# Plachtaa/FAcodec

Hardware: NVIDIA B200
Metric: audio_seconds_per_second (higher is better)
Workload: dtype f32 I/O and accumulation; every product is a 3-MMA split of fp32 operands: fp16 hi + 2^11-scaled fp16 lo (22 mantissa bits, register-promoted accumulation) upstream of the VQ, bf16 hi + bf16 lo (16 bits) downstream

## Files before the change

facodec_b200/csrc/engine.cu:

```cuda
#include <cmath>
#include <cstdio>
#include <cstdlib>
#include <cstring>
#include <map>
#include <string>
#include <vector>

#include "../../include/facodec_b200.h"
#include "../../include/facodec_b200_debug.h"
#include "common.cuh"
#include "kernels.h"

using namespace fac;

namespace {

constexpr int HOP = 300;
constexpr int LATENT = 1024;
constexpr int N_FFT = 2048;
constexpr int WIN = 1200;
constexpr int N_BINS = 1025;
constexpr int SPEC_LD = 2052;
constexpr int SPEC_TC_LD = 2176;
constexpr int N_MELS = 80;

struct HostTensor {
    std::vector<float> data;
    std::vector<int64_t> shape;
    size_t numel() const { size_t n = 1; for (auto s : shape) n *= (size_t)s; return n; }
};

struct ConvW {
    size_t w = 0, b = 0; int Cin = 0, Cout = 0, K = 1, ldw = 0;
    bool tc = false; size_t tcw = 0; int vf = 1, Kr = 0, tcN = 0;
    bool promoted = false;
    bool has16 = false; size_t tcw16 = 0;
    bool has_f16s = false; size_t tcw_f16s = 0;
    bool has_tt = false; size_t tcw_tt = 0;
};
struct SnakeW { size_t a = 0, ia = 0; int C = 0; };
struct LstmW { ConvW ih[2]; size_t whh[2] = {0, 0}; size_t whh16[2] = {0, 0}; bool has16 = false; int H = 0, U = 0, G = 0;
               size_t whh2[2][2] = {{0, 0}, {0, 0}}; bool has2[2] = {false, false}; };
struct ResW { SnakeW s1; ConvW c7; SnakeW s2; ConvW c1; int dil = 1; };
struct VqW { size_t w_in, b_in, cb, cbn, cbn2, w_out, b_out; };

struct EncW {
    ConvW conv0;
    struct Block { ResW res[3]; SnakeW snake; ConvW down; int stride; } blk[4];
    LstmW lstm; SnakeW snake; ConvW conv_out;
};
struct DecW {
    ConvW conv0; LstmW lstm;
    struct Block { SnakeW snake; ConvW up; int stride; int cout; ResW res[3]; } blk[4];
    SnakeW snake; ConvW conv_out;
    bool causal = true, has_lstm = true;
};
struct RedW {
    size_t emb_p = 0, emb_c[2] = {0, 0};
    ConvW cond, wn_in[16], wn_rs[16], conv_out;
    int hidden = 512, layers = 16;
};
struct QuantW {
    VqW vq[6];
    ConvW spec0, spec3, glu[2], cq, ck, cv, co, fc, timbre_linear;
    ConvW mel_lin, wn_in[8], wn_rs[8], mel_lin2;
    ConvW dft; size_t fb = 0;
    ConvW dft_tc;
};
struct RvqSet { int nq; VqW vq[8]; };

}

struct fac_handle {
    int device = 0;
    std::string err;
    std::map<std::string, HostTensor> host[FAC_NUM_MODULES];
    bool have[FAC_NUM_MODULES] = {false, false, false, false, false};
    bool finalized = false;
    std::vector<float> pack;
    float* warena = nullptr; size_t wfloats = 0;
    EncW enc; DecW dec; QuantW qw;
    RedW red; DecW dec2;
    std::vector<RvqSet> rvqs; std::vector<float*> rvq_arenas;
    struct Stream;
    std::vector<Stream*> streams;
    struct HeadSet;
    std::vector<HeadSet*> heads;
    char* ws = nullptr; size_t ws_bytes = 0;
    int launches = 0;
    int use_tc = 2;
    int fuse_res = 1;
    int lstm_v2 = 1;
    int dec_lstm_fp16 = 1;
    int enc_mufu = 0;
    int attn_stream = 0;
    int dec_c7_f16 = 1;
    int enc_tt = 1;
    int enc_f16 = 0;
    int tc_occ2 = 256;
    bool dec_bf16 = true;
    int overlap_front = 1; cudaStream_t side = nullptr; cudaEvent_t ev_fork = nullptr, ev_join = nullptr;
    float* aa_filter = nullptr;
    float* mel16_arena = nullptr; ConvW mel16_dft, mel16_dft_tc; size_t mel16_fb = 0;
    struct LossScale { ConvW dft; size_t fb = 0; int s = 0, nfft = 0, nb = 0, ld = 0; };
    float* loss_arena = nullptr; LossScale loss_scale[6];
    struct SpecScale { ConvW dft; size_t fb = 0; int w = 0, nb = 0, ld = 0, n_out = 0; bool mel = false; };
    float* spec_arena = nullptr; std::vector<SpecScale> spec_scales; std::vector<double> spec_key;
    bool profiling = false;
    struct ProfRec { std::string name; cudaEvent_t a, b; double flops, bytes; };
    std::vector<ProfRec> prof;
    struct ProfAgg { double ms = 0, flops = 0, bytes = 0; long launches = 0; };
    std::map<std::string, ProfAgg> prof_agg;
    std::map<std::string, std::pair<float*, size_t>> taps;
};

struct fac_handle::Stream {
    int B = 0;
    bool alive = false;
    long long enc_samples = 0, dec_frames = 0;
    float* x_hist = nullptr; int x_hist_len = 0;
    float* ey_hist = nullptr; int ey_hist_len = 0;
    float* z_hist = nullptr; int z_hist_len = 0;
    float* dy_hist = nullptr; int dy_hist_len = 0;
    uint32_t* enc_h[2] = {nullptr, nullptr}; float* enc_c[2] = {nullptr, nullptr};
    uint32_t* dec_h[2] = {nullptr, nullptr}; float* dec_c[2] = {nullptr, nullptr};
    void* all[12] = {nullptr};
};

struct fac_handle::HeadSet {
    int indim = 0, outdim = 0, nheads = 0, global_pred = 0;
    struct Unit { size_t a1, b1, a2, b2; ConvW c7, c1; int dil; } unit[3];
    size_t af, bf;
    ConvW lin[8];
    std::map<std::string, HostTensor> staged;
    float* arena = nullptr;
    bool ready = false;
};

namespace {

size_t pack_alloc(fac_handle* h, size_t n) {
    size_t off = (h->pack.size() + 63) / 64 * 64;
    h->pack.resize(off + n, 0.f);
    return off;
}

const HostTensor* find(fac_handle* h, int m, const std::string& k) {
    auto it = h->host[m].find(k);
    return it == h->host[m].end() ? nullptr : &it->second;
}

struct PackError { std::string msg; };
const HostTensor& need(fac_handle* h, int m, const std::string& k) {
    const HostTensor* t = find(h, m, k);
    if (!t) throw PackError{"missing tensor '" + k + "' in module " + std::to_string(m)};
    return *t;
}

std::vector<float> folded_weight(fac_handle* h, int m, const std::string& prefix, std::vector<int64_t>& shape) {
    if (const HostTensor* w = find(h, m, prefix + ".weight")) {
        shape = w->shape;
        return w->data;
    }
    const HostTensor& v = need(h, m, prefix + ".weight_v");
    const HostTensor& g = need(h, m, prefix + ".weight_g");
    shape = v.shape;
    size_t d0 = (size_t)v.shape[0], inner = v.numel() / d0;
    if (g.numel() != d0) throw PackError{"weight_g shape mismatch at " + prefix};
    std::vector<float> w(v.numel());
    for (size_t i = 0; i < d0; ++i) {
        double s = 0.0;
        for (size_t j = 0; j < inner; ++j) { double x = v.data[i * inner + j]; s += x * x; }
        float scale = g.data[i] / (float)std::sqrt(s);
        for (size_t j = 0; j < inner; ++j) w[i * inner + j] = v.data[i * inner + j] * scale;
    }
// ... 491 lines not shown
    p.res = o.res; p.valid_len = o.valid_len;
    p.B = B; p.Tin = Tin; p.Cin = w.Cin; p.Tout = Tout; p.Cout = w.Cout;
    p.K = w.K; p.dil = o.dil; p.stride = o.stride;
    p.pad_left = o.pad_left; p.pad_right = o.pad_right; p.pad_reflect = o.reflect;
    p.ldw = w.ldw; p.ldy = o.ldy ? o.ldy : w.Cout; p.ldx = o.ldx ? o.ldx : w.Cin;
    p.y_transposed = o.transposed;
    p.x_bstride = (size_t)Tin * p.ldx;
    p.y_bstride = (size_t)Tout * p.ldy;
    double flops = 2.0 * B * Tout * (double)w.Cout * w.K * w.Cin;
    double bytes = 4.0 * ((double)B * Tin * w.Cin + (double)B * Tout * w.Cout * (o.res ? 2 : 1) + (double)w.K * w.Cin * w.Cout);
    char det[96];
    snprintf(det, sizeof det, "%s Cin%d Cout%d K%d d%d T%d", name, w.Cin, w.Cout, w.K, o.dil, Tout);
    c.begin("conv", flops, bytes, det);
    c.check(launch_conv(p, c.st), name);
    c.end();
}

int sconv(Ctx& c, const ConvW& w, const float* x, float* y, int B, int T, int dil, int stride, ConvOpts o,
          const char* name, bool causal = true) {
    int k_eff = (w.K - 1) * dil + 1;
    o.dil = dil; o.stride = stride;
    const int total = k_eff - stride, extra = conv_extra_pad(T, k_eff, stride);
    o.pad_left = causal ? total : total - total / 2;
    o.pad_right = (causal ? 0 : total / 2) + extra;
    o.reflect = 1;
    int Tout = conv_out_len(T, k_eff, stride);
    run_conv(c, w, x, y, B, T, Tout, o, name);
    return Tout;
}

bool residual_unit_fused(Ctx& c, const ResW& r, const float* x, float* y, int B, int T, bool causal) {
    if (c.h->use_tc < 1 || !c.h->fuse_res || c.vq_critical || !r.c7.tc || !r.c1.tc || r.c7.promoted || r.c1.promoted ||
        r.c7.Cin != r.c7.Cout || r.c1.K != 1 || r.c7.vf != 1)
        return false;
    TcConvParams tp;
    tp.Cin = r.c7.Cin; tp.Cout = r.c7.Cout; tp.vf = 1; tp.Kr = r.c7.K; tp.dil = r.dil; tp.fused = 1;
    tp.bf16 = (c.h->dec_bf16 && r.c7.has16 && r.c1.has16) ? 1 : 0;
    tp.g1f16 = (tp.bf16 && r.c7.has_f16s && c.h->dec_c7_f16) ? 1 : 0;
    tp.occ2_maxn = c.h->tc_occ2;
    tp.Tout = T;
    if (c.h->fuse_res == 2 && r.c7.Cout > 128) return false;
    if (!tc_conv_plan(tp)) return false;
    if (c.dry) return true;
    const int k_eff = (r.c7.K - 1) * r.dil + 1;
    tp.x = x; tp.y = y; tp.res = x;
    tp.wblob = c.W(tp.g1f16 ? r.c7.tcw_f16s : (tp.bf16 ? r.c7.tcw16 : r.c7.tcw)); tp.bias = c.W(r.c7.b);
    tp.wblob2 = c.W(tp.bf16 ? r.c1.tcw16 : r.c1.tcw); tp.bias2 = c.W(r.c1.b);
    tp.in_alpha = c.W(r.s1.a); tp.in_inv_alpha = c.W(r.s1.ia);
    tp.out_act = ACT_SNAKE; tp.out_alpha = c.W(r.s2.a); tp.out_inv_alpha = c.W(r.s2.ia);
    tp.B = B; tp.Tin = T; tp.ldx = r.c7.Cin;
    const int pl = causal ? k_eff - 1 : (k_eff - 1) - (k_eff - 1) / 2;
    tp.PLr = pl; tp.pad_left_s = pl; tp.pad_right_s = k_eff - 1 - pl; tp.reflect = 1;
    tp.Tout = T; tp.ldy = r.c7.Cout;
    tp.x_bstride = (size_t)T * r.c7.Cin; tp.y_bstride = (size_t)T * r.c7.Cout;
    double flops = 2.0 * B * T * (double)r.c7.Cout * r.c7.Cin * (r.c7.K + 1);
    double bytes = 4.0 * ((double)B * T * r.c7.Cin * 2 + (double)B * T * r.c7.Cout + (double)(r.c7.K + 1) * r.c7.Cin * r.c7.Cout);
    char det[96];
    snprintf(det, sizeof det, "res.fused C%d K%d d%d T%d", r.c7.Cin, r.c7.K, r.dil, T);
    c.begin("conv_tc", flops, bytes, det);
    c.check(launch_conv_tc(tp, c.st), "res.fused");
    c.end();
    return true;
}

void residual_unit(Ctx& c, const ResW& r, const float* x, float* tmp, float* y, int B, int T, bool causal = true) {
    if (residual_unit_fused(c, r, x, y, B, T, causal)) return;
    ConvOpts o1;
    o1.in_snake = &r.s1;
    o1.out_snake = &r.s2;
    sconv(c, r.c7, x, tmp, B, T, r.dil, 1, o1, "res.conv7", causal);
    ConvOpts o2;
    o2.res = x;
    sconv(c, r.c1, tmp, y, B, T, 1, 1, o2, "res.conv1", causal);
}

struct LstmState { uint32_t* h[2] = {nullptr, nullptr}; float* c[2] = {nullptr, nullptr}; };

void slstm(Ctx& c, const LstmW& L, const float* x, float* y, int B, int T, LstmState* st = nullptr) {
    const int H = L.H;
    float* xg = c.alloc<float>((size_t)B * T * 4 * H);
    float* h1 = c.alloc<float>((size_t)B * T * H);
    float* hT = c.alloc<float>((size_t)2 * H * 32);
    uint32_t* h16 = c.alloc<uint32_t>((size_t)2 * 2 * (H / 2) * 32);
    unsigned int* bar = c.alloc<unsigned int>(64);
    for (int l = 0; l < 2; ++l) {
        const float* in = l == 0 ? x : h1;
        ConvOpts o;
        run_conv(c, L.ih[l], in, xg, 1, B * T, B * T, o, "lstm.ih");
        if (c.dry) continue;
        const int pass3 = (c.vq_critical || !c.h->dec_bf16) ? 1 : 0;
        const bool v2 = c.h->lstm_v2 && L.has2[pass3] && (pass3 || c.h->dec_lstm_fp16);
        for (int b0 = 0; b0 < B; b0 += 32) {
            int nb = B - b0 < 32 ? B - b0 : 32;
            LstmParams p;
            p.xg = xg + (size_t)b0 * T * 4 * H;
            p.whh_p = c.W(L.whh[l]);
            if (c.h->dec_bf16 && L.has16 && !c.vq_critical) { p.bf16 = 1; p.whh_p16 = c.W(L.whh16[l]); }
            p.skip = l == 1 ? x + (size_t)b0 * T * H : nullptr;
            p.y = (l == 0 ? h1 : y) + (size_t)b0 * T * H;
            p.hT = hT; p.bar = bar;
            p.B = nb; p.T = T; p.H = H; p.U = L.U; p.G = L.G;
            c.begin("lstm_rec", 2.0 * nb * T * 4.0 * H * H, 4.0 * ((double)nb * T * 5 * H + 4.0 * H * H));
            if (st && (!v2 || B > 32)) { c.check(cudaErrorNotSupported, "lstm.stream (needs the resident-W kernel and B <= 32)"); c.end(); continue; }
            if (v2) {
                p.whh_p2 = reinterpret_cast<const uint32_t*>(c.W(L.whh2[l][pass3]));
                p.h16 = h16; p.pass3 = pass3;
                if (st) { p.state_h = st->h[l]; p.state_c = st->c[l]; }
                c.check(launch_lstm2_layer(p, c.st), "lstm.rec2");
            } else {
                c.check(launch_lstm_layer(p, c.st), "lstm.rec");
            }
            c.end();
        }
    }
}

size_t enc_stage_floats(int B, int T) {
    return (size_t)B * ((size_t)T + 16) * 64;
}

float* encoder_front(Ctx& c, const float* x, int B, int T, int* frames) {
    const EncW& e = c.h->enc;
    size_t stage = enc_stage_floats(B, T);
    float* buf[3] = {c.alloc<float>(stage), c.alloc<float>(stage), c.alloc<float>(stage)};
    int cur = 0;
    int t = sconv(c, e.conv0, x, buf[0], B, T, 1, 1, ConvOpts(), "enc.conv0");
    c.tap("enc_conv0", buf[0], (size_t)B * t * 64);
    static const char* blk_names[4] = {"enc_block1", "enc_block2", "enc_block3", "enc_block4"};
    for (int i = 0; i < 4; ++i) {
        for (int j = 0; j < 3; ++j) {
            int tmp = (cur + 1) % 3, nxt = (cur + 2) % 3;
            residual_unit(c, e.blk[i].res[j], buf[cur], buf[tmp], buf[nxt], B, t);
            cur = nxt;
        }
        ConvOpts o;
        o.in_snake = &e.blk[i].snake;
        int nxt = (cur + 1) % 3;
        t = sconv(c, e.blk[i].down, buf[cur], buf[nxt], B, t, 1, e.blk[i].stride, o, "enc.down");
        cur = nxt;
        c.tap(blk_names[i], buf[cur], (size_t)B * t * e.blk[i].down.Cout);
    }
    *frames = t;
    return buf[cur];
}

int encoder_forward(Ctx& c, const float* x, int B, int T, float* z_out, bool z_nct) {
    const EncW& e = c.h->enc;
    c.vq_critical = true;
    int t = 0;
    float* feats = encoder_front(c, x, B, T, &t);
    float* ylstm = c.alloc<float>((size_t)B * t * LATENT);
    slstm(c, e.lstm, feats, ylstm, B, t);
    c.tap("enc_lstm", ylstm, (size_t)B * t * 1024);
    ConvOpts o;
    o.in_snake = &e.snake;
    if (z_nct) {
        float* zcl = c.alloc<float>((size_t)B * t * LATENT);
        sconv(c, e.conv_out, ylstm, zcl, B, t, 1, 1, o, "enc.conv_out");
        if (!c.dry) c.check(launch_transpose(zcl, z_out, B, t, LATENT, c.st), "enc.z_T");
    } else {
        sconv(c, e.conv_out, ylstm, z_out, B, t, 1, 1, o, "enc.conv_out");
    }
    c.vq_critical = false;
    return t;
}

size_t decoder_stage_floats(int B, int Tf) {
    size_t stage = (size_t)B * (size_t)Tf * 28800 + 1024;
    size_t first = (size_t)B * Tf * 1536;
    return first > stage ? first : stage;
}
void decoder_stack(Ctx& c, const DecW& d, const float* in, int in_idx, float* const* buf, int B, int Tf, float* y) {
    int t = Tf;
    const float* cur_p = in;
    int cur = in_idx;
    static const char* dblk_names[4] = {"dec_block1", "dec_block2", "dec_block3", "dec_block4"};
    for (int i = 0; i < 4; ++i) {
        ConvOpts o;
        o.in_snake = &d.blk[i].snake;
        o.pad_left = 1; o.pad_right = d.causal ? 0 : 1; o.reflect = 0;
        int nxt = cur < 0 ? 0 : (cur + 1) % 3;
        run_conv(c, d.blk[i].up, cur_p, buf[nxt], B, t, t, o, "dec.up");
        cur = nxt; cur_p = buf[cur];
        t *= d.blk[i].stride;
        for (int j = 0; j < 3; ++j) {
            int tmp = (cur + 1) % 3, nx2 = (cur + 2) % 3;
            residual_unit(c, d.blk[i].res[j], buf[cur], buf[tmp], buf[nx2], B, t, d.causal);
            cur = nx2; cur_p = buf[cur];
        }
// ... 1150 lines not shown
        auto i0 = [](double v) { double s = 1, t = 1; for (int k = 1; k < 60; ++k) { t *= (v / (2 * k)) * (v / (2 * k)); s += t; } return s; };
        float f[12];
        double sum = 0;
        double tmp[12];
        for (int i = 0; i < ks; ++i) {
            double r = 2.0 * i / (ks - 1) - 1.0;
            double w = i0(beta_k * std::sqrt(std::max(0.0, 1 - r * r))) / i0(beta_k);
            double tm = (i - half) + 0.5;
            double xx = 2 * cutoff * tm;
            double sinc = xx == 0 ? 1.0 : std::sin(M_PI * xx) / (M_PI * xx);
            tmp[i] = 2 * cutoff * w * sinc;
            sum += tmp[i];
        }
        for (int i = 0; i < ks; ++i) f[i] = (float)(tmp[i] / sum);
        cudaError_t e = cudaMalloc(&h->aa_filter, sizeof(f));
        if (e == cudaSuccess) e = cudaMemcpy(h->aa_filter, f, sizeof(f), cudaMemcpyHostToDevice);
        if (e != cudaSuccess) { h->err = cudaGetErrorString(e); cudaGetLastError(); return FAC_ERR_CUDA; }
    }
    return FAC_OK;
}

int fac_alias_free_act(fac_handle* h, const float* x, int B, int C, int T, int act, const float* alpha,
                       const float* beta, float* y, void* stream) {
    if (!h || !x || !y || B <= 0 || C <= 0 || T <= 0 || (act == 1 && (!alpha || !beta))) return FAC_ERR_INVALID;
    int rc0 = ensure_aa_filter(h);
    if (rc0) return rc0;
    cudaError_t e = launch_alias_free_act(x, y, B, C, T, h->aa_filter, act == 1 ? alpha : nullptr, act == 1 ? beta : nullptr,
                                          (cudaStream_t)stream);
    if (e != cudaSuccess) { h->err = cudaGetErrorString(e); return FAC_ERR_CUDA; }
    return FAC_OK;
}

int fac_debug_conv(fac_handle* h, const float* x, const float* w_host, const float* bias_host, int B, int Tin, int Cin,
                   int Cout, int K, int dil, int stride, int pad_left, int pad_right, int reflect,
                   const float* in_alpha_host, const float* out_alpha_host, int act, const float* res, float* y,
                   int Tout, void* stream) {
    if (!h || !x || !w_host || !y) return FAC_ERR_INVALID;
    cudaSetDevice(h->device);
    cudaStream_t st = (cudaStream_t)stream;
    int ldw = (Cout + 3) / 4 * 4;
    std::vector<float> pk((size_t)K * Cin * ldw + Cout + 2 * Cin + 2 * Cout + 96, 0.f);
    for (int co = 0; co < Cout; ++co)
        for (int ci = 0; ci < Cin; ++ci)
            for (int k = 0; k < K; ++k) pk[((size_t)k * Cin + ci) * ldw + co] = w_host[((size_t)co * Cin + ci) * K + k];
    auto al4 = [](size_t v) { return (v + 3) / 4 * 4; };
    size_t o_b = (size_t)K * Cin * ldw, o_ia = al4(o_b + Cout), o_iia = al4(o_ia + Cin), o_oa = al4(o_iia + Cin), o_oia = al4(o_oa + Cout);
    for (int i = 0; i < Cout; ++i) pk[o_b + i] = bias_host ? bias_host[i] : 0.f;
    for (int i = 0; i < Cin; ++i) { pk[o_ia + i] = in_alpha_host ? in_alpha_host[i] : 1.f; pk[o_iia + i] = 1.0f / (pk[o_ia + i] + 1e-9f); }
    for (int i = 0; i < Cout; ++i) { pk[o_oa + i] = out_alpha_host ? out_alpha_host[i] : 1.f; pk[o_oia + i] = 1.0f / (pk[o_oa + i] + 1e-9f); }
    float* d = nullptr;
    cudaError_t e = cudaMalloc(&d, pk.size() * sizeof(float));
    if (e == cudaSuccess) e = cudaMemcpy(d, pk.data(), pk.size() * sizeof(float), cudaMemcpyHostToDevice);
    if (e != cudaSuccess) { h->err = cudaGetErrorString(e); cudaGetLastError(); return FAC_ERR_CUDA; }
    ConvParams p;
    p.x = x; p.y = y; p.w = d; p.bias = bias_host ? d + o_b : nullptr;
    if (in_alpha_host) { p.in_alpha = d + o_ia; p.in_inv_alpha = d + o_iia; }
    p.out_act = act;
    if (out_alpha_host) { p.out_act = ACT_SNAKE; p.out_alpha = d + o_oa; p.out_inv_alpha = d + o_oia; }
    p.res = res;
    p.B = B; p.Tin = Tin; p.Cin = Cin; p.Tout = Tout; p.Cout = Cout; p.K = K; p.dil = dil; p.stride = stride;
    p.pad_left = pad_left; p.pad_right = pad_right; p.pad_reflect = reflect;
    p.ldw = ldw; p.ldy = Cout; p.ldx = Cin;
    p.x_bstride = (size_t)Tin * Cin; p.y_bstride = (size_t)Tout * Cout;
    e = launch_conv(p, st);
    if (e == cudaSuccess) e = cudaStreamSynchronize(st);
    cudaFree(d);
    if (e != cudaSuccess) { h->err = std::string("fac_debug_conv: ") + cudaGetErrorString(e); return FAC_ERR_CUDA; }
    return FAC_OK;
}

int fac_debug_slstm(fac_handle* h, const float* x, const float* const* w_host, int B, int T, int H, float* y, void* stream) {
    if (!h || !x || !w_host || !y || B <= 0 || T <= 0) return FAC_ERR_INVALID;
    fac_handle tmp;
    tmp.device = h->device;
    const char* names[8] = {"weight_ih_l0", "weight_hh_l0", "bias_ih_l0", "bias_hh_l0", "weight_ih_l1", "weight_hh_l1", "bias_ih_l1", "bias_hh_l1"};
    for (int i = 0; i < 8; ++i) {
        HostTensor t;
        bool mat = (i % 4) < 2;
        if (mat) t.shape = {4 * H, H}; else t.shape = {4 * H};
        t.data.assign(w_host[i], w_host[i] + t.numel());
        tmp.host[0][std::string("l.") + names[i]] = std::move(t);
    }
    tmp.dec_bf16 = h->dec_bf16;
    tmp.lstm_v2 = h->lstm_v2; tmp.dec_lstm_fp16 = h->dec_lstm_fp16;
    LstmW L;
    try { L = pack_lstm(&tmp, 0, "l"); } catch (const PackError& e) { h->err = e.msg; return FAC_ERR_UNSUPPORTED; }
    cudaSetDevice(h->device);
    cudaError_t e = cudaMalloc(&tmp.warena, (tmp.pack.size() + 64) * sizeof(float));
    if (e == cudaSuccess) e = cudaMemcpy(tmp.warena, tmp.pack.data(), tmp.pack.size() * sizeof(float), cudaMemcpyHostToDevice);
    if (e != cudaSuccess) { h->err = cudaGetErrorString(e); cudaGetLastError(); return FAC_ERR_CUDA; }
    cudaStream_t st = (cudaStream_t)stream;
    Ctx dry{&tmp, st, true};
    slstm(dry, L, x, y, B, T);
    int rc = ensure_ws(&tmp, dry.off);
    if (rc == FAC_OK) {
        Ctx c{&tmp, st, false};
        slstm(c, L, x, y, B, T);
        rc = finish(&tmp, c);
        cudaStreamSynchronize(st);
    }
    if (rc != FAC_OK) h->err = tmp.err;
    cudaFree(tmp.warena);
    if (tmp.ws) cudaFree(tmp.ws);
    return rc;
}

int fac_set_option(fac_handle* h, const char* name, int value) {
    if (!h || !name) return FAC_ERR_INVALID;
    if (std::string(name) == "fuse_resunit") { h->fuse_res = value < 0 ? 0 : (value > 2 ? 2 : value); return FAC_OK; }
    if (std::string(name) == "tc_dbg") { g_tc_dbg = value; return FAC_OK; }
    if (std::string(name) == "tc_slot_issue") { g_tc_slot_issue = value != 0; return FAC_OK; }
    if (std::string(name) == "tt_pair") { g_tt_pair_ok = value != 0; return FAC_OK; }
    if (std::string(name) == "tc_groups") { g_tc_groups_ok = value != 0; return FAC_OK; }
    if (std::string(name) == "tc_wide") { g_tc_wide_ok = value != 0; return FAC_OK; }
    if (std::string(name) == "tc_occ2_maxn") { h->tc_occ2 = value < 0 ? 0 : value; return FAC_OK; }
    if (std::string(name) == "encoder_f16x2") { h->enc_f16 = value != 0; return FAC_OK; }
    if (std::string(name) == "decoder_conv7_fp16") { h->dec_c7_f16 = value != 0; return FAC_OK; }
    if (std::string(name) == "encoder_tt") { h->enc_tt = value != 0; return FAC_OK; }
    if (std::string(name) == "encoder_snake_mufu") { h->enc_mufu = value != 0; return FAC_OK; }
    if (std::string(name) == "overlap_front") { h->overlap_front = value != 0; return FAC_OK; }
    if (std::string(name) == "lstm_v2") { h->lstm_v2 = value != 0; return FAC_OK; }
    if (std::string(name) == "decoder_lstm_fp16") { h->dec_lstm_fp16 = value != 0; return FAC_OK; }
    if (std::string(name) == "tt_probe") { g_tt_probe_on = value != 0; return FAC_OK; }
    if (std::string(name) == "attention_stream") { h->attn_stream = value != 0; return FAC_OK; }
    if (std::string(name) == "decoder_bf16") { h->dec_bf16 = value != 0; return FAC_OK; }
    if (std::string(name) == "tensor_cores") { h->use_tc = value < 0 ? 0 : (value > 2 ? 2 : value); return FAC_OK; }
    h->err = std::string("unknown option ") + name;
    return FAC_ERR_INVALID;
}

int fac_debug_conv_tc(fac_handle* h, const float* x, const float* w_host, const float* bias_host, int B, int Tin, int Cin,
                      int Cout, int K, int dil, int stride, int pad_left, int pad_right, int reflect,
                      const float* in_alpha_host, const float* out_alpha_host, int act, const float* res, float* y,
                      int Tout, int promoted, void* stream) {
    if (!h || !x || !w_host || !y) return FAC_ERR_INVALID;
    cudaSetDevice(h->device);
    cudaStream_t st = (cudaStream_t)stream;
    TcConvParams tp;
    tp.Cin = Cin; tp.Cout = Cout; tp.promoted = (promoted == 1 || promoted == 3) ? 1 : 0; tp.bf16 = (promoted == 2 || promoted == 5) ? 1 : 0;
    tp.f16x2 = promoted == 3 ? 1 : 0;
    tp.g1f16 = promoted == 5 ? 1 : 0;
    const bool use_tt = promoted == 4;
    tp.occ2_maxn = h->tc_occ2;
    tp.Tout = Tout;
    if (stride == 1) { tp.vf = 1; tp.Kr = K; tp.dil = dil; }
    else if (K == 2 * stride && dil == 1) { tp.vf = stride; tp.Kr = 2; tp.dil = 1; }
    else { h->err = "fac_debug_conv_tc: unsupported stride/kernel"; return FAC_ERR_UNSUPPORTED; }
    if (!(use_tt ? tt_conv_plan(tp) : tc_conv_plan(tp))) { h->err = "fac_debug_conv_tc: layer not eligible for the tensor-core path"; return FAC_ERR_UNSUPPORTED; }
    int ldw = (Cout + 3) / 4 * 4;
    std::vector<float> gen((size_t)K * Cin * ldw, 0.f);
    for (int co = 0; co < Cout; ++co)
        for (int ci = 0; ci < Cin; ++ci)
            for (int k = 0; k < K; ++k) gen[((size_t)k * Cin + ci) * ldw + co] = w_host[((size_t)co * Cin + ci) * K + k];
    size_t nb = use_tt ? tt_blob_floats(tp) : tc_blob_floats(tp);
    auto al4 = [](size_t v) { return (v + 3) / 4 * 4; };
    size_t o_b = al4(nb), o_ia = al4(o_b + Cout), o_iia = al4(o_ia + Cin), o_oa = al4(o_iia + Cin), o_oia = al4(o_oa + Cout);
    std::vector<float> pk(o_oia + Cout + 16, 0.f);
    if (use_tt) tt_pack_blob(tp, gen.data(), ldw, pk.data());
    else tc_pack_blob(tp, gen.data(), ldw, pk.data());
    for (int i = 0; i < Cout; ++i) pk[o_b + i] = bias_host ? bias_host[i] : 0.f;
    for (int i = 0; i < Cin; ++i) { pk[o_ia + i] = in_alpha_host ? in_alpha_host[i] : 1.f; pk[o_iia + i] = 1.0f / (pk[o_ia + i] + 1e-9f); }
    for (int i = 0; i < Cout; ++i) { pk[o_oa + i] = out_alpha_host ? out_alpha_host[i] : 1.f; pk[o_oia + i] = 1.0f / (pk[o_oa + i] + 1e-9f); }
    float* d = nullptr;
    cudaError_t e = cudaMalloc(&d, pk.size() * sizeof(float));
    if (e == cudaSuccess) e = cudaMemcpy(d, pk.data(), pk.size() * sizeof(float), cudaMemcpyHostToDevice);
    if (e != cudaSuccess) { h->err = cudaGetErrorString(e); cudaGetLastError(); return FAC_ERR_CUDA; }
    tp.x = x; tp.y = y; tp.wblob = d; tp.bias = d + o_b;
    if (in_alpha_host) { tp.in_alpha = d + o_ia; tp.in_inv_alpha = d + o_iia; }
    tp.out_act = act;
    if (out_alpha_host) { tp.out_act = ACT_SNAKE; tp.out_alpha = d + o_oa; tp.out_inv_alpha = d + o_oia; }
    tp.res = res;
    tp.B = B; tp.Tin = Tin; tp.ldx = Cin;
    tp.PLr = pad_left / tp.vf;
    tp.pad_left_s = pad_left; tp.pad_right_s = pad_right; tp.reflect = reflect;
    tp.Tout = Tout; tp.ldy = Cout;
    tp.x_bstride = (size_t)Tin * Cin; tp.y_bstride = (size_t)Tout * Cout;
    e = use_tt ? launch_conv_tt(tp, st) : launch_conv_tc(tp, st);
    if (e == cudaSuccess) e = cudaStreamSynchronize(st);
    cudaFree(d);
    if (e != cudaSuccess) { h->err = std::string("fac_debug_conv_tc: ") + cudaGetErrorString(e); return FAC_ERR_CUDA; }
    return FAC_OK;
}

int fac_debug_resunit(fac_handle* h, const float* x, const float* w7_host, const float* b7_host, const float* w1_host,
                      const float* b1_host, const float* alpha1_host, const float* alpha2_host, int B, int T, int C,
                      int dil, int mode, float* y, void* stream) {
    if (!h || !x || !y || !w7_host || !w1_host) return FAC_ERR_INVALID;
    fac_handle tmp;
    tmp.device = h->device;
    tmp.use_tc = mode == 0 ? 0 : 1;
    tmp.fuse_res = (mode == 2 || mode == 4 || mode == 6) ? 1 : 0;
    tmp.dec_bf16 = mode >= 3;
    tmp.dec_c7_f16 = mode >= 5;
    tmp.tc_occ2 = h->tc_occ2;
    auto put = [&](const char* key, const float* d, std::vector<int64_t> shp) {
        HostTensor t;
        t.shape = shp;
        t.data.assign(d, d + t.numel());
        tmp.host[0][key] = std::move(t);
    };
    put("u.block.0.alpha", alpha1_host, {1, C, 1});
    put("u.block.1.conv.conv.weight", w7_host, {C, C, 7});
    put("u.block.1.conv.conv.bias", b7_host, {C});
    put("u.block.2.alpha", alpha2_host, {1, C, 1});
// ... 244 lines not shown
```

facodec_b200/csrc/kernels.h:

```cpp
#pragma once
#include <cuda_runtime.h>
#include <stdint.h>

namespace fac {

struct ConvParams {
    const float* x = nullptr;
    const float* w = nullptr;
    const float* bias = nullptr;
    const float* in_alpha = nullptr;
    const float* in_inv_alpha = nullptr;
    const float* out_alpha = nullptr;
    const float* out_inv_alpha = nullptr;
    const float* res = nullptr;
    const int* valid_len = nullptr;
    float* y = nullptr;
    int B = 0, Tin = 0, Cin = 0, Tout = 0, Cout = 0;
    int K = 1, dil = 1, stride = 1, pad_left = 0, pad_right = 0, pad_reflect = 0;
    int ldw = 0, ldy = 0, ldx = 0;
    int out_act = 0;
    int y_transposed = 0;
    size_t x_bstride = 0, y_bstride = 0;
};
cudaError_t launch_conv(const ConvParams& p, cudaStream_t st);

struct TcConvParams {
    const float* x = nullptr;
    const float* wblob = nullptr;
    const float* bias = nullptr;
    const float* in_alpha = nullptr;
    const float* in_inv_alpha = nullptr;
    const float* out_alpha = nullptr;
    const float* out_inv_alpha = nullptr;
    const float* res = nullptr;
    float* y = nullptr;
    int B = 0, Tin = 0, Cin = 0, ldx = 0;
    int vf = 1;
    int Kr = 1, dil = 1, PLr = 0;
    int pad_left_s = 0, pad_right_s = 0, reflect = 0;
    int Tout = 0, Cout = 0, ldy = 0;
    int out_act = 0;
    int promoted = 0;
    int bf16 = 0;
    int g1f16 = 0;
    int f16x2 = 0;
    int tt = 0;
    int pair = 0;
    int NT = 0;
    int snake_mufu = 0;
    int fused = 0;
    const float* wblob2 = nullptr;
    const float* bias2 = nullptr;
    int nchunk2 = 0;
    int occ2_maxn = 0;
    int promote_every = 1;
    int N = 0, MT = 0, nchunk = 0, Rpad = 0, stagesB = 0, tmem_cols = 0;
    int cps = 0;
    int tpt = 1, tpt2 = 1;
    int b_slot = 0;
    int R2pad = 0;
    int dbg = 0;
    int ng = 1;
    int wide = 0;
    size_t smem_bytes = 0;
    size_t x_bstride = 0, y_bstride = 0;
};
bool tc_conv_plan(TcConvParams& p);
size_t tc_blob_floats(const TcConvParams& p);
void tc_pack_blob(const TcConvParams& p, const float* wp, int ldw, float* blob);
cudaError_t launch_conv_tc(const TcConvParams& p, cudaStream_t st);
bool tt_conv_plan(TcConvParams& p);
size_t tt_blob_floats(const TcConvParams& p);
void tt_pack_blob(const TcConvParams& p, const float* wp, int ldw, float* blob);
cudaError_t launch_conv_tt(const TcConvParams& p, cudaStream_t st);
extern int g_tc_dbg;
extern int g_tc_slot_issue;
extern int g_tc_groups_ok;
extern int g_tc_wide_ok;
extern int g_tt_pair_ok;
extern int g_tt_probe_on;
cudaError_t tt_read_probe(long long* out8);
cudaError_t tc_read_trace(long long* out80);
cudaError_t tc_read_producer_clocks(long long* out4);
cudaError_t tc_read_phase_clocks(long long* out8);

struct LstmParams {
    const float* xg = nullptr;
    const float* whh_p = nullptr;
    const float* whh_p16 = nullptr;
    int bf16 = 0;
    const uint32_t* whh_p2 = nullptr;
    uint32_t* h16 = nullptr;
    int pass3 = 0;
    uint32_t* state_h = nullptr;
    float* state_c = nullptr;
    const float* skip = nullptr;
    float* y = nullptr;
    float* hT = nullptr;
    unsigned int* bar = nullptr;
    int B = 0, T = 0, H = 0, U = 0, G = 0;
};
cudaError_t launch_lstm_layer(const LstmParams& p, cudaStream_t st);
cudaError_t launch_lstm2_layer(const LstmParams& p, cudaStream_t st);
size_t lstm2_pack_words(int H, int U, int pass3);
void lstm2_pack(const float* whh, int H, int U, int pass3, uint32_t* out);
size_t lstm2_smem_bytes(int H, int U, int pass3);
cudaError_t lstm2_read_phase_clocks(long long* out4);
int lstm_units_per_cta(int H);
cudaError_t lstm_read_phase_clocks(long long* out4);

cudaError_t launch_stft_frames(const float* wave, float* frames , int B, int T, int F, int hop, int win, int pad,
                               cudaStream_t st);
cudaError_t launch_mel_from_spec(const float* spec, int ldspec, const float* fb , float* mel,
                                 int B, int F, int Tm, cudaStream_t st);

struct VqWeights {
    const float* w_in;
    const float* b_in;
    const float* cb;
    const float* cbn;
    const float* cbn2;
    const float* w_out;
    const float* b_out;
};
struct FaqParams {
    const float* f0 = nullptr;
    const float* z = nullptr;
    VqWeights vq[6];
    int n_c = 1;
    const float* gamma_beta = nullptr;
    float* outs = nullptr;
    float* zp = nullptr, *zc = nullptr, *zr = nullptr;
    int64_t* codes_p = nullptr;
    int64_t* codes_c = nullptr;
    int64_t* codes_r = nullptr;
    float* sqerr = nullptr;
    int B = 0, Tq = 0, Tz = 0, Tf0 = 0;
};
cudaError_t launch_fa_quantize(const FaqParams& p, cudaStream_t st);
cudaError_t launch_vq_loss_reduce(const float* sqerr, int nq, int B, int Tq, float* losses2, cudaStream_t st);

struct RvqParams {
    const float* x = nullptr;
    VqWeights vq[8];
    int nq = 0;
    float* qout = nullptr;
    float* allq = nullptr;
    int64_t* idx = nullptr;
    int B = 0, T = 0;
};
cudaError_t launch_rvq(const RvqParams& p, cudaStream_t st);

cudaError_t launch_mel_loss_terms(const float* spec, int ldspec, int nb, const float* fb , int B, int F, float eps,
                                  float* terms , cudaStream_t st);
cudaError_t launch_strided_sum(const float* in, long long n, int stride, double scale, double* out, cudaStream_t st);
cudaError_t launch_sqdiff_partial(const float* a, const float* b, long long n, float* part, int nblocks, cudaStream_t st);
cudaError_t launch_spec_loss_terms(const float* spec, int ldspec, int nb, const float* fb , int n_out, int B, int F,
                                   float eps, float pw, float* terms , cudaStream_t st);
cudaError_t launch_absdiff_partial(const float* a, const float* b, long long n, float* part, int nblocks, cudaStream_t st);
cudaError_t launch_spec_loss_combine(const double* v, int n, float mag_weight, float log_weight, float* loss, cudaStream_t st);
cudaError_t launch_add3(const float* a, const float* b, const float* c , long long n, float* out, cudaStream_t st);
cudaError_t launch_loss_combine(const double* v13, float* loss, float* terms, cudaStream_t st);
cudaError_t launch_transpose(const float* in, float* out, int B, int R, int C, cudaStream_t st);
cudaError_t launch_wn_gate(const float* xin, float* acts, size_t n_rows, int hidden, cudaStream_t st, const float* g = nullptr,
                           size_t rows_per_utt = 0, size_t g_stride = 0);
cudaError_t launch_wn_update(const float* rs, float* x, float* out, size_t n_rows, int hidden, int last, cudaStream_t st);
cudaError_t launch_glu_res(const float* y, float* x, int B, int T, int C, const int* valid_len, cudaStream_t st);
cudaError_t launch_attention(const float* q, const float* k, const float* v, float* o, int B, int T, int heads,
                             int dk, const int* valid_len, cudaStream_t st, int force_stream = 0);
cudaError_t launch_mean_pool(const float* x, float* out, int B, int T, int C, const int* valid_len, cudaStream_t st);
cudaError_t launch_fill_u32(unsigned int* p, unsigned int v, size_t n, cudaStream_t st);

cudaError_t launch_alias_free_act(const float* x, float* y, int B, int C, int T, const float* filt12,
                                  const float* alpha, const float* inv_beta, cudaStream_t st);

}
// ... 1 lines not shown
```

facodec_b200/csrc/lstm2.cu:

```cuda
#include <cooperative_groups.h>
#include <cuda_fp16.h>

#include <cstring>

#include "common.cuh"
#include "kernels.h"

namespace fac {

__device__ long long g_lstm2_phase_clock[4];

namespace {
constexpr int L2_BT = 32;
constexpr int L2_WARPS = 8;
template <bool PASS3> struct L2Depth { static constexpr int D = PASS3 ? 4 : 8; };

__device__ __forceinline__ void mma_f16_16x8x16(float (&d)[4], const uint32_t (&a)[4], const uint32_t (&b)[2]) {
    asm volatile(
        "mma.sync.aligned.m16n8k16.row.col.f32.f16.f16.f32 {%0,%1,%2,%3}, {%4,%5,%6,%7}, {%8,%9}, {%0,%1,%2,%3};"
        : "+f"(d[0]), "+f"(d[1]), "+f"(d[2]), "+f"(d[3])
        : "r"(a[0]), "r"(a[1]), "r"(a[2]), "r"(a[3]), "r"(b[0]), "r"(b[1]));
}
__device__ __forceinline__ void cp16(void* smem, const void* gmem) {
    unsigned s = (unsigned)__cvta_generic_to_shared(smem);
    asm volatile("cp.async.cg.shared.global [%0], [%1], 16;\n" ::"r"(s), "l"(gmem));
}
__device__ __forceinline__ void cp_commit() { asm volatile("cp.async.commit_group;\n" ::); }
template <int N>
__device__ __forceinline__ void cp_wait() { asm volatile("cp.async.wait_group %0;\n" ::"n"(N)); }
}

__host__ __device__ __forceinline__ int lstm2_swz_w(int k2, int R) { return R == 32 ? ((k2 & 3) << 3) : (((k2 >> 1) & 1) << 3); }
__host__ __device__ __forceinline__ int lstm2_swz_h(int kp) { return (kp & 3) << 3; }

template <int U, bool PASS3>
__global__ void __launch_bounds__(L2_WARPS * 32, 1) lstm_rec2_kernel(LstmParams p) {
    constexpr int R = 4 * U;
    constexpr int RP = R + 1;
    constexpr int MT = R / 16, NTL = L2_BT / 8;
    constexpr int PL = PASS3 ? 2 : 1;
    constexpr int L2_DEPTH = L2Depth<PASS3>::D;
    constexpr int STAGE_W = PL * 8 * L2_BT;
    static_assert(L2_DEPTH * STAGE_W >= L2_BT * RP, "reduction buffer must fit in a warp's own stage memory");
    extern __shared__ __align__(16) uint32_t smem2[];
    const int H = p.H;
    const int nsub_all = H / 16;
    uint32_t* wres = smem2;
    uint32_t* stage_base = wres + (size_t)nsub_all * PL * 8 * R;
    float* cstate = reinterpret_cast<float*>(stage_base + L2_WARPS * L2_DEPTH * STAGE_W);

    const int tid = threadIdx.x, warp = tid >> 5, lane = tid & 31;
    const int cta = blockIdx.x;
    const int j0 = cta * U;
    const int nsub = nsub_all / L2_WARPS;
    const int sub0 = warp * nsub;
    const int fg = lane >> 2, ft = lane & 3;

    {
        const uint4* src = reinterpret_cast<const uint4*>(p.whh_p2 + (size_t)cta * nsub_all * PL * 8 * R);
        uint4* dst = reinterpret_cast<uint4*>(wres);
        const int n16 = nsub_all * PL * 8 * R / 4;
        for (int i = tid; i < n16; i += blockDim.x) dst[i] = __ldg(src + i);
    }
    for (int i = tid; i < L2_BT * U; i += blockDim.x) cstate[i] = p.state_c ? p.state_c[(size_t)cta * L2_BT * U + i] : 0.f;
    __syncthreads();

    uint32_t* my_stage = stage_base + warp * L2_DEPTH * STAGE_W;
    const size_t plane_words = (size_t)(H / 2) * L2_BT;
    constexpr int PAIRS = (L2_BT * U + L2_WARPS * 32 - 1) / (L2_WARPS * 32);
    const bool probe = (cta == 0 && tid == 0);
    long long ph[4] = {0, 0, 0, 0}, tc0 = 0;

    for (int t = 0; t < p.T; ++t) {
        if (probe) tc0 = clock64();
        float xgv[PAIRS][4];
        float skv[PAIRS];
#pragma unroll
        for (int pi = 0; pi < PAIRS; ++pi) {
            int idx = tid + pi * L2_WARPS * 32;
            int b = idx % L2_BT, u = idx / L2_BT;
            skv[pi] = (p.skip && idx < L2_BT * U && b < p.B) ? __ldg(p.skip + ((size_t)b * p.T + t) * H + j0 + u) : 0.f;
#pragma unroll
            for (int g = 0; g < 4; ++g)
                xgv[pi][g] = (idx < L2_BT * U && b < p.B) ? __ldg(p.xg + ((size_t)b * p.T + t) * (4 * H) + (size_t)g * H + j0 + u) : 0.f;
        }
        if (t > 0) {
            if (tid == 0) {
                unsigned target = (unsigned)p.G * (unsigned)t;
                unsigned v;
                long long w0 = clock64();
                do {
                    asm volatile("ld.acquire.gpu.global.u32 %0, [%1];\n" : "=r"(v) : "l"(p.bar));
                    if (v < target && clock64() - w0 > 4000000000LL) __trap();
                } while (v < target);
            }
            __syncthreads();
        }
        const uint32_t* hprev = p.h16 + (size_t)((t + 1) & 1) * PL * plane_words;
        if (probe) { long long n = clock64(); ph[0] += n - tc0; tc0 = n; }

        float acc0[MT][NTL][4];
        float acc1[PASS3 ? MT : 1][PASS3 ? NTL : 1][4];
#pragma unroll
        for (int i = 0; i < MT; ++i)
#pragma unroll
            for (int j = 0; j < NTL; ++j)
#pragma unroll
                for (int e = 0; e < 4; ++e) { acc0[i][j][e] = 0.f; if (PASS3) acc1[i][j][e] = 0.f; }

        auto issue_h = [&](int sub) {
            uint32_t* hs = my_stage + (sub % L2_DEPTH) * STAGE_W;
#pragma unroll
            for (int pl = 0; pl < PL; ++pl) {
                const uint32_t* hg = hprev + pl * plane_words + (size_t)(sub0 + sub) * 8 * L2_BT;
#pragma unroll
                for (int i = lane; i < 8 * L2_BT / 4; i += 32) cp16(hs + pl * 8 * L2_BT + i * 4, hg + i * 4);
            }
        };
#pragma unroll
        for (int s0 = 0; s0 < L2_DEPTH - 1; ++s0) {
            if (s0 < nsub) issue_h(s0);
            cp_commit();
        }
        for (int sub = 0; sub < nsub; ++sub) {
            const int nxt = sub + L2_DEPTH - 1;
            if (nxt < nsub) issue_h(nxt);
            cp_commit();
            cp_wait<L2_DEPTH - 1>();
            __syncwarp();
            const uint32_t* hs = my_stage + (sub % L2_DEPTH) * STAGE_W;
            const uint32_t* wh = wres + (size_t)(sub0 + sub) * PL * 8 * R;
            uint32_t bh[NTL][2], bl[PASS3 ? NTL : 1][2];
#pragma unroll
            for (int j = 0; j < NTL; ++j) {
                const int c0 = (j * 8 + fg) ^ lstm2_swz_h(ft);
                bh[j][0] = hs[ft * L2_BT + c0];
                bh[j][1] = hs[(ft + 4) * L2_BT + c0];
                if (PASS3) {
                    bl[j][0] = hs[8 * L2_BT + ft * L2_BT + c0];
                    bl[j][1] = hs[8 * L2_BT + (ft + 4) * L2_BT + c0];
                }
            }
            const int sw = lstm2_swz_w(ft, R);
#pragma unroll
            for (int i = 0; i < MT; ++i) {
                uint32_t ah[4], al[4];
                const int r0 = (i * 16 + fg) ^ sw, r1 = (i * 16 + fg + 8) ^ sw;
                ah[0] = wh[ft * R + r0];        ah[1] = wh[ft * R + r1];
                ah[2] = wh[(ft + 4) * R + r0];  ah[3] = wh[(ft + 4) * R + r1];
                if (PASS3) {
                    al[0] = wh[8 * R + ft * R + r0];        al[1] = wh[8 * R + ft * R + r1];
                    al[2] = wh[8 * R + (ft + 4) * R + r0];  al[3] = wh[8 * R + (ft + 4) * R + r1];
                }
#pragma unroll
                for (int j = 0; j < NTL; ++j) {
                    mma_f16_16x8x16(acc0[i][j], ah, bh[j]);
                    if (PASS3) {
                        mma_f16_16x8x16(acc1[i][j], ah, bl[j]);
                        mma_f16_16x8x16(acc1[i][j], al, bh[j]);
                    }
                }
            }
            __syncwarp();
        }
        if (probe) { long long n = clock64(); ph[1] += n - tc0; tc0 = n; }
        float* myred = reinterpret_cast<float*>(my_stage);
#pragma unroll
        for (int i = 0; i < MT; ++i)
#pragma unroll
            for (int j = 0; j < NTL; ++j) {
                const int r0 = i * 16 + fg, b0 = j * 8 + 2 * ft;
                float v0 = acc0[i][j][0], v1 = acc0[i][j][1], v2 = acc0[i][j][2], v3 = acc0[i][j][3];
                if (PASS3) {
                    v0 = fmaf(acc1[i][j][0], 1.0f / 2048.0f, v0); v1 = fmaf(acc1[i][j][1], 1.0f / 2048.0f, v1);
                    v2 = fmaf(acc1[i][j][2], 1.0f / 2048.0f, v2); v3 = fmaf(acc1[i][j][3], 1.0f / 2048.0f, v3);
                }
                myred[b0 * RP + r0] = v0;
                myred[(b0 + 1) * RP + r0] = v1;
                myred[b0 * RP + r0 + 8] = v2;
                myred[(b0 + 1) * RP + r0 + 8] = v3;
            }
        __syncthreads();

        __half* hcur = reinterpret_cast<__half*>(p.h16 + (size_t)(t & 1) * PL * plane_words);
#pragma unroll
        for (int pi = 0; pi < PAIRS; ++pi) {
            int idx = tid + pi * L2_WARPS * 32;
            if (idx >= L2_BT * U) break;
            int b = idx % L2_BT, u = idx / L2_BT;
            float g4[4];
#pragma unroll
            for (int g = 0; g < 4; ++g) {
                float s = 0.f;
#pragma unroll
                for (int w = 0; w < L2_WARPS; ++w)
                    s += reinterpret_cast<const float*>(stage_base + w * L2_DEPTH * STAGE_W)[b * RP + g * U + u];
                g4[g] = s + xgv[pi][g];
            }
            float ig = sigmoid_f(g4[0]), fgt = sigmoid_f(g4[1]), gg = tanhf(g4[2]), og = sigmoid_f(g4[3]);
            float c = fgt * cstate[b * U + u] + ig * gg;
            cstate[b * U + u] = c;
            float h = og * tanhf(c);
            const int k = j0 + u, kp = k >> 1;
            const size_t widx = (size_t)kp * L2_BT + (size_t)(b ^ lstm2_swz_h(kp));
            const __half hh = __float2half_rn(h);
            hcur[widx * 2 + (k & 1)] = hh;
            if (PASS3) hcur[(plane_words + widx) * 2 + (k & 1)] = __float2half_rn((h - __half2float(hh)) * 2048.0f);
            if (b < p.B) {
                size_t o = ((size_t)b * p.T + t) * H + j0 + u;
                p.y[o] = h + skv[pi];
            }
        }
        if (probe) { long long n = clock64(); ph[2] += n - tc0; tc0 = n; }
        __syncthreads();
        if (tid == 0) {
            __threadfence();
            atomicAdd(p.bar, 1u);
        }
        if (probe) { long long n = clock64(); ph[3] += n - tc0; }
    }
    if (p.state_c) {
        __syncthreads();
        for (int i = tid; i < L2_BT * U; i += blockDim.x) p.state_c[(size_t)cta * L2_BT * U + i] = cstate[i];
    }
    if (probe) { for (int i = 0; i < 4; ++i) g_lstm2_phase_clock[i] = ph[i]; }
}

cudaError_t lstm2_read_phase_clocks(long long* out4) { return cudaMemcpyFromSymbol(out4, g_lstm2_phase_clock, sizeof(long long) * 4); }

size_t lstm2_pack_words(int H, int U, int pass3) { return (size_t)(H / U) * (H / 16) * (pass3 ? 2 : 1) * 8 * (4 * U); }
void lstm2_pack(const float* whh, int H, int U, int pass3, uint32_t* out) {
    const int G = H / U, R = 4 * U, PL = pass3 ? 2 : 1;
    auto bits = [](__half v) { uint16_t b; memcpy(&b, &v, 2); return (uint32_t)b; };
    for (int cta = 0; cta < G; ++cta)
        for (int sub = 0; sub < H / 16; ++sub)
            for (int k2 = 0; k2 < 8; ++k2)
                for (int r = 0; r < R; ++r) {
                    const int g = r / U, u = r % U;
                    const float* wrow = &whh[((size_t)g * H + cta * U + u) * H + sub * 16 + 2 * k2];
                    const __half h0 = __float2half_rn(wrow[0]), h1 = __float2half_rn(wrow[1]);
                    const size_t base = (((size_t)cta * (H / 16) + sub) * PL) * 8 * R;
                    const int col = r ^ lstm2_swz_w(k2, R);
                    out[base + (size_t)k2 * R + col] = bits(h0) | (bits(h1) << 16);
                    if (pass3) {
                        const __half l0 = __float2half_rn((wrow[0] - __half2float(h0)) * 2048.0f);
                        const __half l1 = __float2half_rn((wrow[1] - __half2float(h1)) * 2048.0f);
                        out[base + (size_t)(8 + k2) * R + col] = bits(l0) | (bits(l1) << 16);
                    }
                }
}

size_t lstm2_smem_bytes(int H, int U, int pass3) {
    const int R = 4 * U, PL = pass3 ? 2 : 1;
    const int depth = pass3 ? 4 : 8;
    return sizeof(uint32_t) * ((size_t)(H / 16) * PL * 8 * R + (size_t)L2_WARPS * depth * PL * 8 * L2_BT) + sizeof(float) * L2_BT * U;
}

template <int U, bool PASS3>
static cudaError_t launch2_u(const LstmParams& p, cudaStream_t st) {
    const size_t smem = lstm2_smem_bytes(p.H, U, PASS3 ? 1 : 0);
    if (smem > 227 * 1024) return cudaErrorInvalidValue;
    cudaError_t e = cudaFuncSetAttribute(lstm_rec2_kernel<U, PASS3>, cudaFuncAttributeMaxDynamicSharedMemorySize, (int)smem);
    if (e != cudaSuccess) return e;
    e = cudaMemsetAsync(p.bar, 0, sizeof(unsigned int), st);
    if (e != cudaSuccess) return e;
    const size_t plane_words = (size_t)(p.H / 2) * L2_BT;
    const int PL = PASS3 ? 2 : 1;
    if (p.state_h) e = cudaMemcpyAsync(p.h16 + (size_t)PL * plane_words, p.state_h, sizeof(uint32_t) * PL * plane_words, cudaMemcpyDeviceToDevice, st);
    else e = cudaMemsetAsync(p.h16 + (size_t)PL * plane_words, 0, sizeof(uint32_t) * PL * plane_words, st);
    if (e != cudaSuccess) return e;
    LstmParams pp = p;
    void* args[] = {&pp};
    e = cudaLaunchCooperativeKernel((void*)lstm_rec2_kernel<U, PASS3>, dim3(p.G), dim3(L2_WARPS * 32), args, smem, st);
    if (e != cudaSuccess) return e;
    if (p.state_h) e = cudaMemcpyAsync(p.state_h, p.h16 + (size_t)((p.T - 1) & 1) * PL * plane_words, sizeof(uint32_t) * PL * plane_words, cudaMemcpyDeviceToDevice, st);
    return e;
}

cudaError_t launch_lstm2_layer(const LstmParams& p, cudaStream_t st) {
    if (p.B > L2_BT || p.B <= 0 || !p.whh_p2 || !p.h16) return cudaErrorInvalidValue;
    if ((p.H / 16) % L2_WARPS != 0) return cudaErrorInvalidValue;
    if (p.U == 8) return p.pass3 ? launch2_u<8, true>(p, st) : launch2_u<8, false>(p, st);
    if (p.U == 12) return p.pass3 ? launch2_u<12, true>(p, st) : launch2_u<12, false>(p, st);
    return cudaErrorInvalidValue;
}

}
```

Measured before the change: 2237.

## Replace LSTM grid-wide barrier with per-CTA release/acquire flags and staged h exchange

The recurrent LSTM kernel no longer waits on one global atomic counter that every CTA increments each timestep. Each CTA now publishes its own timestep flag with a release store, and each warp acquire-polls only the flags of the CTAs that produce the h slice it consumes. The new h values are staged in shared memory and copied out as 16-byte vector stores before the flag is published. The reduction buffer layout is transposed for float2 stores, and output writes are moved after the publish. This is meant to cut per-step grid synchronization latency on the sequential critical path, at the cost of more flag polling traffic and a bit more shared memory.

```diff
diff --git a/facodec_b200/csrc/engine.cu b/facodec_b200/csrc/engine.cu
--- a/facodec_b200/csrc/engine.cu
+++ b/facodec_b200/csrc/engine.cu
@@ -91,6 +91,7 @@
     int use_tc = 2;
     int fuse_res = 1;
     int lstm_v2 = 1;
+    int lstm_xchg = 1;
     int dec_lstm_fp16 = 1;
     int enc_mufu = 0;
     int attn_stream = 0;
@@ -748,7 +749,7 @@
     float* h1 = c.alloc<float>((size_t)B * T * H);
     float* hT = c.alloc<float>((size_t)2 * H * 32);
     uint32_t* h16 = c.alloc<uint32_t>((size_t)2 * 2 * (H / 2) * 32);
-    unsigned int* bar = c.alloc<unsigned int>(64);
+    unsigned int* bar = c.alloc<unsigned int>(L.G > 64 ? L.G : 64);
     for (int l = 0; l < 2; ++l) {
         const float* in = l == 0 ? x : h1;
         ConvOpts o;
@@ -770,7 +771,7 @@
             if (st && (!v2 || B > 32)) { c.check(cudaErrorNotSupported, "lstm.stream (needs the resident-W kernel and B <= 32)"); c.end(); continue; }
             if (v2) {
                 p.whh_p2 = reinterpret_cast<const uint32_t*>(c.W(L.whh2[l][pass3]));
-                p.h16 = h16; p.pass3 = pass3;
+                p.h16 = h16; p.pass3 = pass3; p.exchange = c.h->lstm_xchg;
                 if (st) { p.state_h = st->h[l]; p.state_c = st->c[l]; }
                 c.check(launch_lstm2_layer(p, c.st), "lstm.rec2");
             } else {
@@ -2087,7 +2088,7 @@
         tmp.host[0][std::string("l.") + names[i]] = std::move(t);
     }
     tmp.dec_bf16 = h->dec_bf16;
-    tmp.lstm_v2 = h->lstm_v2; tmp.dec_lstm_fp16 = h->dec_lstm_fp16;
+    tmp.lstm_v2 = h->lstm_v2; tmp.dec_lstm_fp16 = h->dec_lstm_fp16; tmp.lstm_xchg = h->lstm_xchg;
     LstmW L;
     try { L = pack_lstm(&tmp, 0, "l"); } catch (const PackError& e) { h->err = e.msg; return FAC_ERR_UNSUPPORTED; }
     cudaSetDevice(h->device);
@@ -2125,6 +2126,7 @@
     if (std::string(name) == "encoder_snake_mufu") { h->enc_mufu = value != 0; return FAC_OK; }
     if (std::string(name) == "overlap_front") { h->overlap_front = value != 0; return FAC_OK; }
     if (std::string(name) == "lstm_v2") { h->lstm_v2 = value != 0; return FAC_OK; }
+    if (std::string(name) == "lstm_exchange") { h->lstm_xchg = value != 0; return FAC_OK; }
     if (std::string(name) == "decoder_lstm_fp16") { h->dec_lstm_fp16 = value != 0; return FAC_OK; }
     if (std::string(name) == "tt_probe") { g_tt_probe_on = value != 0; return FAC_OK; }
     if (std::string(name) == "attention_stream") { h->attn_stream = value != 0; return FAC_OK; }
diff --git a/facodec_b200/csrc/kernels.h b/facodec_b200/csrc/kernels.h
--- a/facodec_b200/csrc/kernels.h
+++ b/facodec_b200/csrc/kernels.h
@@ -92,6 +92,7 @@
     const uint32_t* whh_p2 = nullptr;
     uint32_t* h16 = nullptr;
     int pass3 = 0;
+    int exchange = 1;
     uint32_t* state_h = nullptr;
     float* state_c = nullptr;
     const float* skip = nullptr;
diff --git a/facodec_b200/csrc/lstm2.cu b/facodec_b200/csrc/lstm2.cu
--- a/facodec_b200/csrc/lstm2.cu
+++ b/facodec_b200/csrc/lstm2.cu
@@ -33,21 +33,30 @@
 __host__ __device__ __forceinline__ int lstm2_swz_w(int k2, int R) { return R == 32 ? ((k2 & 3) << 3) : (((k2 >> 1) & 1) << 3); }
 __host__ __device__ __forceinline__ int lstm2_swz_h(int kp) { return (kp & 3) << 3; }
 
-template <int U, bool PASS3>
+__device__ __forceinline__ unsigned ld_acquire_u32(const unsigned* a) {
+    unsigned v;
+    asm volatile("ld.acquire.gpu.global.u32 %0, [%1];\n" : "=r"(v) : "l"(a) : "memory");
+    return v;
+}
+
+template <int U, bool PASS3, bool XCHG>
 __global__ void __launch_bounds__(L2_WARPS * 32, 1) lstm_rec2_kernel(LstmParams p) {
     constexpr int R = 4 * U;
     constexpr int RP = R + 1;
+    constexpr int BP = L2_BT + 8;
     constexpr int MT = R / 16, NTL = L2_BT / 8;
     constexpr int PL = PASS3 ? 2 : 1;
     constexpr int L2_DEPTH = L2Depth<PASS3>::D;
     constexpr int STAGE_W = PL * 8 * L2_BT;
-    static_assert(L2_DEPTH * STAGE_W >= L2_BT * RP, "reduction buffer must fit in a warp's own stage memory");
+    static_assert(L2_DEPTH * STAGE_W >= L2_BT * RP && L2_DEPTH * STAGE_W >= R * BP, "reduction buffer must fit in a warp's own stage memory");
+    static_assert(U % 2 == 0, "a k pair of h must belong to one CTA");
     extern __shared__ __align__(16) uint32_t smem2[];
     const int H = p.H;
     const int nsub_all = H / 16;
     uint32_t* wres = smem2;
     uint32_t* stage_base = wres + (size_t)nsub_all * PL * 8 * R;
     float* cstate = reinterpret_cast<float*>(stage_base + L2_WARPS * L2_DEPTH * STAGE_W);
+    uint32_t* hstage = reinterpret_cast<uint32_t*>(cstate + L2_BT * U);
 
     const int tid = threadIdx.x, warp = tid >> 5, lane = tid & 31;
     const int cta = blockIdx.x;
@@ -55,6 +64,7 @@
     const int nsub = nsub_all / L2_WARPS;
     const int sub0 = warp * nsub;
     const int fg = lane >> 2, ft = lane & 3;
+    const int prod_lo = sub0 * 16 / U, prod_hi = ((sub0 + nsub) * 16 - 1) / U;
 
     {
         const uint4* src = reinterpret_cast<const uint4*>(p.whh_p2 + (size_t)cta * nsub_all * PL * 8 * R);
@@ -84,7 +94,15 @@
             for (int g = 0; g < 4; ++g)
                 xgv[pi][g] = (idx < L2_BT * U && b < p.B) ? __ldg(p.xg + ((size_t)b * p.T + t) * (4 * H) + (size_t)g * H + j0 + u) : 0.f;
         }
-        if (t > 0) {
+        if (XCHG && t > 0) {
+            for (int c = prod_lo + lane; c <= prod_hi; c += 32) {
+                long long w0 = clock64();
+                while (ld_acquire_u32(p.bar + c) < (unsigned)t)
+                    if (clock64() - w0 > 4000000000LL) __trap();
+            }
+            __syncwarp();
+        }
+        if (!XCHG && t > 0) {
             if (tid == 0) {
                 unsigned target = (unsigned)p.G * (unsigned)t;
                 unsigned v;
@@ -175,14 +193,20 @@
                     v0 = fmaf(acc1[i][j][0], 1.0f / 2048.0f, v0); v1 = fmaf(acc1[i][j][1], 1.0f / 2048.0f, v1);
                     v2 = fmaf(acc1[i][j][2], 1.0f / 2048.0f, v2); v3 = fmaf(acc1[i][j][3], 1.0f / 2048.0f, v3);
                 }
-                myred[b0 * RP + r0] = v0;
-                myred[(b0 + 1) * RP + r0] = v1;
-                myred[b0 * RP + r0 + 8] = v2;
-                myred[(b0 + 1) * RP + r0 + 8] = v3;
+                if (XCHG) {
+                    *reinterpret_cast<float2*>(myred + r0 * BP + b0) = make_float2(v0, v1);
+                    *reinterpret_cast<float2*>(myred + (r0 + 8) * BP + b0) = make_float2(v2, v3);
+                } else {
+                    myred[b0 * RP + r0] = v0;
+                    myred[(b0 + 1) * RP + r0] = v1;
+                    myred[b0 * RP + r0 + 8] = v2;
+                    myred[(b0 + 1) * RP + r0 + 8] = v3;
+                }
             }
         __syncthreads();
 
         __half* hcur = reinterpret_cast<__half*>(p.h16 + (size_t)(t & 1) * PL * plane_words);
+        float yv[PAIRS];
 #pragma unroll
         for (int pi = 0; pi < PAIRS; ++pi) {
             int idx = tid + pi * L2_WARPS * 32;
@@ -194,7 +218,7 @@
                 float s = 0.f;
 #pragma unroll
                 for (int w = 0; w < L2_WARPS; ++w)
-                    s += reinterpret_cast<const float*>(stage_base + w * L2_DEPTH * STAGE_W)[b * RP + g * U + u];
+                    s += reinterpret_cast<const float*>(stage_base + w * L2_DEPTH * STAGE_W)[XCHG ? (g * U + u) * BP + b : b * RP + g * U + u];
                 g4[g] = s + xgv[pi][g];
             }
             float ig = sigmoid_f(g4[0]), fgt = sigmoid_f(g4[1]), gg = tanhf(g4[2]), og = sigmoid_f(g4[3]);
@@ -204,16 +228,44 @@
             const int k = j0 + u, kp = k >> 1;
             const size_t widx = (size_t)kp * L2_BT + (size_t)(b ^ lstm2_swz_h(kp));
             const __half hh = __float2half_rn(h);
-            hcur[widx * 2 + (k & 1)] = hh;
-            if (PASS3) hcur[(plane_words + widx) * 2 + (k & 1)] = __float2half_rn((h - __half2float(hh)) * 2048.0f);
-            if (b < p.B) {
-                size_t o = ((size_t)b * p.T + t) * H + j0 + u;
-                p.y[o] = h + skv[pi];
+            const __half hl = __float2half_rn((h - __half2float(hh)) * 2048.0f);
+            if (XCHG) {
+                __half* hs = reinterpret_cast<__half*>(hstage);
+                const int wl = (int)widx - (j0 / 2) * L2_BT;
+                hs[wl * 2 + (k & 1)] = hh;
+                if (PASS3) hs[((U / 2) * L2_BT + wl) * 2 + (k & 1)] = hl;
+                yv[pi] = h + skv[pi];
+            } else {
+                hcur[widx * 2 + (k & 1)] = hh;
+                if (PASS3) hcur[(plane_words + widx) * 2 + (k & 1)] = hl;
+                if (b < p.B) {
+                    size_t o = ((size_t)b * p.T + t) * H + j0 + u;
+                    p.y[o] = h + skv[pi];
+                }
             }
         }
         if (probe) { long long n = clock64(); ph[2] += n - tc0; tc0 = n; }
         __syncthreads();
-        if (tid == 0) {
+        if (XCHG) {
+            if (warp == 0) {
+                constexpr int SLICE4 = (U / 2) * L2_BT / 4;
+                const uint4* src = reinterpret_cast<const uint4*>(hstage);
+#pragma unroll
+                for (int i = lane; i < PL * SLICE4; i += 32) {
+                    const int pl = i / SLICE4, q = i % SLICE4;
+                    uint4* dst = reinterpret_cast<uint4*>(reinterpret_cast<uint32_t*>(hcur) + pl * plane_words + (size_t)(j0 / 2) * L2_BT);
+                    dst[q] = src[i];
+                }
+                __syncwarp();
+                if (lane == 0) asm volatile("st.release.gpu.global.u32 [%0], %1;\n" ::"l"(p.bar + cta), "r"((unsigned)(t + 1)) : "memory");
+            }
+#pragma unroll
+            for (int pi = 0; pi < PAIRS; ++pi) {
+                int idx = tid + pi * L2_WARPS * 32;
+                int b = idx % L2_BT, u = idx / L2_BT;
+                if (idx < L2_BT * U && b < p.B) p.y[((size_t)b * p.T + t) * H + j0 + u] = yv[pi];
+            }
+        } else if (tid == 0) {
             __threadfence();
             atomicAdd(p.bar, 1u);
         }
@@ -253,16 +305,18 @@
 size_t lstm2_smem_bytes(int H, int U, int pass3) {
     const int R = 4 * U, PL = pass3 ? 2 : 1;
     const int depth = pass3 ? 4 : 8;
-    return sizeof(uint32_t) * ((size_t)(H / 16) * PL * 8 * R + (size_t)L2_WARPS * depth * PL * 8 * L2_BT) + sizeof(float) * L2_BT * U;
+    return sizeof(uint32_t) * ((size_t)(H / 16) * PL * 8 * R + (size_t)L2_WARPS * depth * PL * 8 * L2_BT + (size_t)PL * (U / 2) * L2_BT) +
+           sizeof(float) * L2_BT * U;
 }
 
 template <int U, bool PASS3>
 static cudaError_t launch2_u(const LstmParams& p, cudaStream_t st) {
     const size_t smem = lstm2_smem_bytes(p.H, U, PASS3 ? 1 : 0);
     if (smem > 227 * 1024) return cudaErrorInvalidValue;
-    cudaError_t e = cudaFuncSetAttribute(lstm_rec2_kernel<U, PASS3>, cudaFuncAttributeMaxDynamicSharedMemorySize, (int)smem);
+    const void* kern = p.exchange ? (const void*)lstm_rec2_kernel<U, PASS3, true> : (const void*)lstm_rec2_kernel<U, PASS3, false>;
+    cudaError_t e = cudaFuncSetAttribute(kern, cudaFuncAttributeMaxDynamicSharedMemorySize, (int)smem);
     if (e != cudaSuccess) return e;
-    e = cudaMemsetAsync(p.bar, 0, sizeof(unsigned int), st);
+    e = cudaMemsetAsync(p.bar, 0, sizeof(unsigned int) * (p.exchange ? p.G : 1), st);
     if (e != cudaSuccess) return e;
     const size_t plane_words = (size_t)(p.H / 2) * L2_BT;
     const int PL = PASS3 ? 2 : 1;
@@ -271,7 +325,7 @@
     if (e != cudaSuccess) return e;
     LstmParams pp = p;
     void* args[] = {&pp};
-    e = cudaLaunchCooperativeKernel((void*)lstm_rec2_kernel<U, PASS3>, dim3(p.G), dim3(L2_WARPS * 32), args, smem, st);
+    e = cudaLaunchCooperativeKernel(kern, dim3(p.G), dim3(L2_WARPS * 32), args, smem, st);
     if (e != cudaSuccess) return e;
     if (p.state_h) e = cudaMemcpyAsync(p.state_h, p.h16 + (size_t)((p.T - 1) & 1) * PL * plane_words, sizeof(uint32_t) * PL * plane_words, cudaMemcpyDeviceToDevice, st);
     return e;
```

Measured after the change: 2072 (median of 6 runs). -7.4%, worse.
